# ahmetaa/fast-dnn

Hardware: AMD Instinct MI355X
Metric: acoustic frames/sec (whole node), 7x2048->8000 nnet (higher is better)
Workload: dtype int8 (u8 activations x s8 weights -> int32; fp32 layer 0 and soft-max)

## Files before the change

### fast-dnn_amd/csrc/fdnn_l0s.hip

```cpp
#include <atomic>
#include <cmath>
#include <cstdlib>
#include <limits>
#include <type_traits>
#include <vector>

#include "fdnn_device.hpp"
#include "fdnn_kernels.hpp"

namespace fdnn {

namespace {

#ifndef FDNN_L0S_DEBUG
#define FDNN_L0S_DEBUG 0
#endif
constexpr float kU = 5.9604645e-8f;
constexpr int kSplitW = 32;

[[maybe_unused]] __device__ __forceinline__ bool split_tile_of_block(int node_tiles, int frame_tiles, int &bx, int &by) {
  const int b = blockIdx.x, xcd = b & 7, slot = b >> 3;
  bx = slot % node_tiles;
  by = xcd + 8 * (slot / node_tiles);
  return by < frame_tiles;
}

constexpr int kDigFrames = 8;
__global__ __launch_bounds__(256) void l0_digits_kernel(L0Params p, int KC, int J, int JP) {
  extern __shared__ __attribute__((aligned(16))) float dig_smem[];
  const int D = p.D, ld = D + 1;
  float *xs = dig_smem;
  float *cf_s = dig_smem + kDigFrames * ld;
  const int tid = threadIdx.x, f0 = blockIdx.x * kDigFrames;
  if (blockIdx.x == 0 && tid < 2) p.glist_count[tid] = 0u;
  const int quads = D >> 2;
  {
    float4 raw[4], sh[4], sc[4];
    int rowq[4];
#pragma unroll
    for (int it = 0; it < 4; ++it) {
      const int i = tid + it * 256;
      const int row = i / quads, q = i - row * quads, f = f0 + row;
      const bool in = i < kDigFrames * quads;
      rowq[it] = in ? row * ld + 4 * q : -1;
      raw[it] = make_float4(0.f, 0.f, 0.f, 0.f);
      sh[it] = raw[it];
      sc[it] = raw[it];
      if (in && f < p.n) {
        raw[it] = *reinterpret_cast<const float4 *>(p.x + static_cast<size_t>(f) * D + 4 * q);
        sh[it] = *reinterpret_cast<const float4 *>(p.shift + 4 * q);
        sc[it] = *reinterpret_cast<const float4 *>(p.scale + 4 * q);
      }
    }
#pragma unroll
    for (int it = 0; it < 4; ++it) {
      if (rowq[it] < 0) continue;
      float *dst = xs + rowq[it];
      dst[0] = (raw[it].x + sh[it].x) * sc[it].x;
      dst[1] = (raw[it].y + sh[it].y) * sc[it].y;
      dst[2] = (raw[it].z + sh[it].z) * sc[it].z;
      dst[3] = (raw[it].w + sh[it].w) * sc[it].w;
    }
  }
  __syncthreads();
  {
    const int row = tid >> 5, sub = tid & 31;
    float mx = 0.0f, s2 = 0.0f, s1 = 0.0f;
    int bad = 0;
    float vals[16];
#pragma unroll
    for (int it = 0; it < 16; ++it) vals[it] = sub + 32 * it < D ? xs[row * ld + sub + 32 * it] : 0.0f;
#pragma unroll
    for (int it = 0; it < 16; ++it) {
      const float v = vals[it], a = fabsf(v);
      bad |= !(a < 3.0e38f);
      mx = fmaxf(mx, a);
      s2 = fmaf(v, v, s2);
      s1 += a;
    }
#pragma unroll
    for (int off = 1; off < 32; off <<= 1) {
      mx = fmaxf(mx, __shfl_xor(mx, off));
      s2 += __shfl_xor(s2, off);
      s1 += __shfl_xor(s1, off);
      bad |= __shfl_xor(bad, off);
    }
    if (sub == 0) {
      const bool degenerate = bad || mx > 1.0e18f || (mx != 0.0f && mx < 1.0e-18f);
      const float cf = (mx == 0.0f || degenerate) ? 1.0f : 8355000.0f / mx;
      cf_s[row] = degenerate ? 0.0f : cf;
      const float fD = static_cast<float>(D);
      const float slack = 1.001f + 2.0f * kU * fD;
      const float n1X = (cf * s1 * slack + fD) * 1.001f;
      const float n1X1 = n1X * (1.0f / 65536.0f) + 0.502f * fD;
      const float m = static_cast<float>(JP / 32 + 1);
      const float a_f = kU * (kSplitW + 3) * m * 0.502f * n1X1 + 2.3283064e-10f * (0.5f * n1X + 0.5f * fD) + kU * 256.0f * fD;
      const int f = f0 + row;
      if (f < p.n_ld) {
        p.xstat[f] = 65536.0f / cf;
        p.xstat[p.n_ld + f] = sqrtf(s2) * (1.00001f + 2.0f * kU * fD);
        p.xstat[2 * p.n_ld + f] = degenerate ? __builtin_inff() : 256.0f * a_f * 1.002f;
      }
    }
  }
  __syncthreads();
  for (int idx = tid; idx < kDigFrames * KC * 2; idx += 256) {
    const int row = idx & 7, hh = (idx >> 3) & 1, kc = idx >> 4;
    const float cf = cf_s[row];
    uint32_t d1[4], d2[4], d3[4];
#pragma unroll
    for (int e4 = 0; e4 < 4; ++e4) {
      uint32_t w1 = 0, w2 = 0, w3 = 0;
#pragma unroll
      for (int e = 0; e < 4; ++e) {
        const int pp = kc * 32 + hh * 16 + e4 * 4 + e;
        const int c = (pp >= JP) + (pp >= 2 * JP) + (pp >= 3 * JP), j = pp - c * JP;
        const float v = j < J ? xs[row * ld + 4 * j + c] : 0.0f;
        const int X = static_cast<int>(rintf(v * cf));
        const int x3 = (X << 24) >> 24, r = (X - x3) >> 8, x2 = (r << 24) >> 24, x1 = (r - x2) >> 8;
        w1 |= static_cast<uint32_t>(x1 & 0xff) << (8 * e);
        w2 |= static_cast<uint32_t>(x2 & 0xff) << (8 * e);
        w3 |= static_cast<uint32_t>(x3 & 0xff) << (8 * e);
      }
      d1[e4] = w1; d2[e4] = w2; d3[e4] = w3;
    }
    const int f = f0 + row;
    if (f >= p.n_ld) continue;
    const size_t blocks = static_cast<size_t>(p.n_ld >> 5);
#pragma unroll
    for (int pl = 0; pl < 3; ++pl) {
      const uint32_t *d = pl == 0 ? d1 : pl == 1 ? d2 : d3;
      char *base = reinterpret_cast<char *>(p.xd) + ((static_cast<size_t>(kc) * 3 + pl) * blocks + (f >> 5)) * 1024 + hh * 512 + (f & 31) * 16;
      *reinterpret_cast<uint4 *>(base) = make_uint4(d[0], d[1], d[2], d[3]);
    }
  }
}

constexpr int kSTF = 128, kSStages = 3;
template <int WN>
struct SplitCfg {
  static constexpr int TN = 64 * WN, NW = 4 * WN, THREADS = 64 * NW;
  static constexpr int PIECES = 12 + 6 * WN;
  static constexpr int STAGE = PIECES * 1024;
  static constexpr int RING = STAGE * kSStages;
  static constexpr int HALF_OFF = RING;
  static constexpr int STAT_OFF = RING + 11 * 1024;
  static constexpr int LDS = STAT_OFF + 3 * 1024;
  static constexpr int TS = TN + 16;
  static constexpr int PPW = (PIECES + NW - 1) / NW;
  static_assert(kSTF * TS + 16 + 2 * kL0ScreenCap <= RING, "epilogue tile and flag list must fit in the dead ring");
};
static_assert(4 * kLut2Size <= 11 * 1024, "half-step table area");

template <int WN, bool DBG = false>
__global__ __launch_bounds__(256 * WN, 3 - WN) void l0_split_kernel(L0Params p, int KC, int CPC) {
#if defined(__HIP_DEVICE_COMPILE__)
  using Cfg = SplitCfg<WN>;
  constexpr int kSTN = Cfg::TN, kSStage = Cfg::STAGE, kSTS = Cfg::TS, kSHalfOff = Cfg::HALF_OFF, kSStatOff = Cfg::STAT_OFF, NW = Cfg::NW;
  extern __shared__ __attribute__((aligned(16))) char smem[];
  const int tid = threadIdx.x, lane = tid & 63;
  const int wave = __builtin_amdgcn_readfirstlane(tid >> 6);
  const int l32 = lane & 31, h = lane >> 5;
  const int wf = wave & 3, wn = wave >> 2;
  const int node_tiles = p.h_ld / kSTN, frame_tiles = (p.n_rows + kSTF - 1) / kSTF;
  int bx, by;
  if (!split_tile_of_block(node_tiles, frame_tiles, bx, by)) return;
  const int f0 = by * kSTF, n0 = bx * kSTN;
  const int xblocks = p.n_ld >> 5, wblocks = p.h_ld >> 5;
#ifdef FDNN_L0S_CLK
  long long tc[12];
  tc[0] = __builtin_readcyclecounter();
#define L0S_TS(i) tc[i] = __builtin_readcyclecounter()
#else
#define L0S_TS(i)
#endif

  {
    const __amdgpu_buffer_rsrc_t rsrc_half =
        __builtin_amdgcn_make_buffer_rsrc(const_cast<uint32_t *>(p.luthalf), 0, (4 * kLut2Size + 15) & ~15, 0x00020000);
#pragma unroll
    for (int i = 0; i < 14; ++i) {
      if (i % NW != wave) continue;
      if (i < 11) {
        __builtin_amdgcn_raw_ptr_buffer_load_lds(rsrc_half, FDNN_LDS_PTR(smem + kSHalfOff + i * 1024), 16, lane * 16, i * 1024, 0, 0);
      } else {
        const int q = i - 11;
        const __amdgpu_buffer_rsrc_t rsrc_st =
            __builtin_amdgcn_make_buffer_rsrc(const_cast<float *>(p.xstat + static_cast<size_t>(q) * p.n_ld + f0), 0, kSTF * 4, 0x00020000);
        __builtin_amdgcn_raw_ptr_buffer_load_lds(rsrc_st, FDNN_LDS_PTR(smem + kSStatOff + q * 1024), 16, lane * 16, 0, 0, 0);
      }
    }
  }
  const __amdgpu_buffer_rsrc_t rsrc_x =
      __builtin_amdgcn_make_buffer_rsrc(const_cast<int8_t *>(p.xd), 0, static_cast<unsigned>(KC) * 3u * static_cast<unsigned>(xblocks) * 1024u, 0x00020000);
  const __amdgpu_buffer_rsrc_t rsrc_w = __builtin_amdgcn_make_buffer_rsrc(
      const_cast<int8_t *>(p.wd), 0, static_cast<unsigned>(KC) * 3u * static_cast<unsigned>(wblocks) * 1024u, 0x00020000);
  const int voff = lane * 16;
  const int my_pieces = (Cfg::PIECES - wave + NW - 1) / NW;
  auto stage_piece = [&](int kc, int buf, int t) {
    char *base = smem + buf * kSStage;
    const int i = wave + NW * t;
    if (i >= Cfg::PIECES) return;
    if (i < 12) {
      const int pl = i >> 2, q = i & 3;
      __builtin_amdgcn_raw_ptr_buffer_load_lds(rsrc_x, FDNN_LDS_PTR(base + i * 1024), 16, voff, ((kc * 3 + pl) * xblocks + (f0 >> 5) + q) * 1024, 0, 0);
    } else {
      const int j = i - 12, pl = j / (2 * WN), q = j % (2 * WN);
      __builtin_amdgcn_raw_ptr_buffer_load_lds(rsrc_w, FDNN_LDS_PTR(base + i * 1024), 16, voff, ((kc * 3 + pl) * wblocks + (n0 >> 5) + q) * 1024, 0, 0);
    }
  };
  auto stage = [&](int kc, int buf) {
#pragma unroll
    for (int t = 0; t < Cfg::PPW; ++t) stage_piece(kc, buf, t);
  };
  auto wait_stages = [&](int stages) {
    if (stages == 0) {
      asm volatile("s_waitcnt vmcnt(0) lgkmcnt(0)" ::: "memory");
    } else if (Cfg::PIECES % NW == 0) {
      if (stages == 1)
        asm volatile("s_waitcnt vmcnt(%0) lgkmcnt(0)" ::"n"(Cfg::PPW) : "memory");
      else
        asm volatile("s_waitcnt vmcnt(%0) lgkmcnt(0)" ::"n"(2 * Cfg::PPW) : "memory");
    } else if (my_pieces == Cfg::PPW) {
      if (stages == 1)
        asm volatile("s_waitcnt vmcnt(%0) lgkmcnt(0)" ::"n"(Cfg::PPW) : "memory");
      else
        asm volatile("s_waitcnt vmcnt(%0) lgkmcnt(0)" ::"n"(2 * Cfg::PPW) : "memory");
    } else {
      if (stages == 1)
        asm volatile("s_waitcnt vmcnt(%0) lgkmcnt(0)" ::"n"(Cfg::PPW - 1) : "memory");
      else
        asm volatile("s_waitcnt vmcnt(%0) lgkmcnt(0)" ::"n"(2 * (Cfg::PPW - 1)) : "memory");
    }
  };
  stage(0, 0);
  stage(1, 1);
  stage(2, 2);
  asm volatile("" ::: "memory");

  constexpr int kP0Off = 0x40000000;
  v16i P0[2], P1[2], P2[2];
  uint32_t A[2][16];
#pragma unroll
  for (int s = 0; s < 2; ++s)
#pragma unroll
    for (int r = 0; r < 16; ++r) {
      P0[s][r] = kP0Off; P1[s][r] = 0; P2[s][r] = 0;
      A[s][r] = 0u;
    }
  auto chain_end = [&](int s) {
#pragma unroll
    for (int r = 0; r < 16; ++r) {
      P1[s][r] += P0[s][r] << 8;
      P0[s][r] = kP0Off;
    }
  };
  v4i xa[2][3], wb[2][3][2];
  auto load_plane = [&](int buf, int set, int pl) {
    const char *sb = smem + buf * kSStage;
    xa[set][pl] = *reinterpret_cast<const v4i *>(sb + (pl * 4 + wf) * 1024 + lane * 16);
#pragma unroll
    for (int s = 0; s < 2; ++s) wb[set][pl][s] = *reinterpret_cast<const v4i *>(sb + 12288 + (pl * 2 * WN + wn * 2 + s) * 1024 + lane * 16);
  };
  auto load_frags = [&](int buf, int set) {
#pragma unroll
    for (int pl = 0; pl < 3; ++pl) load_plane(buf, set, pl);
  };
  auto sample_part = [&](int ss, int r0, int r1, bool on) {
    if ((FDNN_L0S_DEBUG & 1) || !on) return;
#pragma unroll
    for (int r = r0; r < r1; ++r) asm volatile("v_sad_u32 %0, %1, 2.0, %0" : "+v"(A[ss][r]) : "v"(P0[ss][r]));
  };
#define FDNN_L0S_FENCE __builtin_amdgcn_sched_barrier(0)
  auto mfma_group = [&](int set, int s, int ss, bool on, auto x0, auto x1, auto x2, auto x3, auto x4) {
    FDNN_L0S_FENCE;
    P0[s] = __builtin_amdgcn_mfma_i32_32x32x32_i8(xa[set][0], wb[set][0][s], P0[s], 0, 0, 0);
    if (FDNN_L0S_DEBUG & 2) {
      sample_part(ss, 0, 16, on);
      x0(); x1(); x2(); x3(); x4();
      return;
    }
    FDNN_L0S_FENCE;
    sample_part(ss, 0, 3, on);
    x0();
    FDNN_L0S_FENCE;
    P1[s] = __builtin_amdgcn_mfma_i32_32x32x32_i8(xa[set][0], wb[set][1][s], P1[s], 0, 0, 0);
    FDNN_L0S_FENCE;
    sample_part(ss, 3, 6, on);
    x1();
    FDNN_L0S_FENCE;
    P2[s] = __builtin_amdgcn_mfma_i32_32x32x32_i8(xa[set][0], wb[set][2][s], P2[s], 0, 0, 0);
    FDNN_L0S_FENCE;
    sample_part(ss, 6, 9, on);
    x2();
    FDNN_L0S_FENCE;
    P1[s] = __builtin_amdgcn_mfma_i32_32x32x32_i8(xa[set][1], wb[set][0][s], P1[s], 0, 0, 0);
    FDNN_L0S_FENCE;
    sample_part(ss, 9, 12, on);
    x3();
    FDNN_L0S_FENCE;
    P2[s] = __builtin_amdgcn_mfma_i32_32x32x32_i8(xa[set][1], wb[set][1][s], P2[s], 0, 0, 0);
    FDNN_L0S_FENCE;
    sample_part(ss, 12, 16, on);
    x4();
    FDNN_L0S_FENCE;
    P2[s] = __builtin_amdgcn_mfma_i32_32x32x32_i8(xa[set][2], wb[set][0][s], P2[s], 0, 0, 0);
    FDNN_L0S_FENCE;
  };
  auto nothing = [] {};

  wait_stages(2);
  __builtin_amdgcn_s_barrier();
  asm volatile("" ::: "memory");
  load_frags(0, 0);
  L0S_TS(1);
  auto chunk = [&](int kc, auto set_c, auto first_c, bool chain_start) {
    constexpr int set = decltype(set_c)::value;
    constexpr bool first = decltype(first_c)::value;
    if (chain_start) chain_end(0);
    mfma_group(set, 0, 1, !first, nothing, nothing, nothing, nothing, nothing);
    const bool more = kc + 1 < KC, refill = kc + 3 < KC && !(FDNN_L0S_DEBUG & 8);
    if (more) {
      wait_stages(kc + 2 < KC ? 1 : 0);
      if (!(FDNN_L0S_DEBUG & 16)) __builtin_amdgcn_s_barrier();
      asm volatile("" ::: "memory");
    }
    if (chain_start) chain_end(1);
    const int nb = (kc + 1) % 3;
    mfma_group(
        set, 1, 0, true, [&] { if (more && !(FDNN_L0S_DEBUG & 32)) load_plane(nb, set ^ 1, 0); if (refill) stage_piece(kc + 3, kc % 3, 0); },
        [&] { if (more && !(FDNN_L0S_DEBUG & 32)) load_plane(nb, set ^ 1, 1); if (refill) stage_piece(kc + 3, kc % 3, 1); },
        [&] { if (more && !(FDNN_L0S_DEBUG & 32)) load_plane(nb, set ^ 1, 2); if (refill) stage_piece(kc + 3, kc % 3, 2); },
        [&] { if (refill && Cfg::PPW > 3) stage_piece(kc + 3, kc % 3, 3); }, [&] { if (refill && Cfg::PPW > 4) stage_piece(kc + 3, kc % 3, 4); });
  };
  using C0 = std::integral_constant<int, 0>;
  using C1 = std::integral_constant<int, 1>;
  chunk(0, C0{}, std::true_type{}, false);
  chunk(1, C1{}, std::false_type{}, false);
  for (int kc = 2, in_chain = 2; kc < KC; kc += 2, in_chain += 2) {
    const bool chain_start = in_chain == CPC;
    if (chain_start) in_chain = 0;
    chunk(kc, C0{}, std::false_type{}, chain_start);
    chunk(kc + 1, C1{}, std::false_type{}, false);
  }
  sample_part(1, 0, 16, true);
  chain_end(0);
  chain_end(1);
  L0S_TS(2);

  __syncthreads();
  const char *half_b = smem + kSHalfOff + 4 * kLut2Half;
  const float *rf_s = reinterpret_cast<const float *>(smem + kSStatOff);
  const float *xn_s = rf_s + 256, *af_s = rf_s + 512;
  uint8_t *tile = reinterpret_cast<uint8_t *>(smem);
  uint32_t *scr_n = reinterpret_cast<uint32_t *>(tile + kSTF * kSTS);
  uint16_t *scr_l = reinterpret_cast<uint16_t *>(tile + kSTF * kSTS + 16);
  if (tid == 0) *scr_n = 0;
  const float fD = static_cast<float>(p.D);
  const float c2 = 1.001f * (0.5f * fD * fD + 2.0f * fD) * kU;
  const float kA = 1.00001f * 256.0f * 1.002f * kU * (kSplitW + 3);
  const float kS = 100.001f * 1.002f * kU * (kSplitW / 2 + 2 + c2);
  float bias100[2], rn100[2], kSw2[2], bn2[2], eb2[2];
  bool node_in[2];
#pragma unroll
  for (int s = 0; s < 2; ++s) {
    const int node = n0 + wn * 64 + s * 32 + l32;
    node_in[s] = node < p.H;
    const float b = node_in[s] ? p.bias[node] : 0.0f;
    bias100[s] = 100.0f * b;
    rn100[s] = 100.0f * (node_in[s] ? p.wstat[node] : 0.0f);
    kSw2[s] = kS * (node_in[s] ? p.wstat[p.h_ld + node] : 0.0f);
    bn2[s] = 1.00001f * (node_in[s] ? p.wstat[2 * p.h_ld + node] : 0.0f);
    eb2[s] = 100.001f * 10.0f * kU * fabsf(b);
  }
  uint32_t valid = 0;
#pragma unroll
  for (int r = 0; r < 16; ++r) {
    const bool row_in = f0 + wf * 32 + 8 * (r >> 2) + 4 * h + (r & 3) < p.n;
    valid |= (row_in && node_in[0] ? 1u : 0u) << r;
    valid |= (row_in && node_in[1] ? 1u : 0u) << (16 + r);
  }
  float tt[2][16], sg[2][16];
  uint32_t ent[2][16];
#pragma unroll
  for (int r = 0; r < 16; ++r) {
    const float rf = rf_s[wf * 32 + 8 * (r >> 2) + 4 * h + (r & 3)];
#pragma unroll
    for (int s = 0; s < 2; ++s) {
      const float v = fmaf(static_cast<float>(P2[s][r]), 0.00390625f, static_cast<float>(P1[s][r]));
      sg[s][r] = rf * rn100[s];
      tt[s][r] = fmaf(v, sg[s][r], bias100[s]);
      const int u = lut2_clamp(static_cast<int>(tt[s][r] + tt[s][r]));
      ent[s][r] = *reinterpret_cast<const uint32_t *>(half_b + 4 * u);
    }
  }
  uint32_t scr_mask = 0;
#pragma unroll
  for (int r = 0; r < 16; ++r) {
    const int row = wf * 32 + 8 * (r >> 2) + 4 * h + (r & 3);
    const float xn = xn_s[row], af = af_s[row];
#pragma unroll
    for (int s = 0; s < 2; ++s) {
      const float t = tt[s][r], sig = sg[s][r];
      tile[row * kSTS + wn * 64 + s * 32 + l32] = static_cast<uint8_t>(ent[s][r]);
      if (!(FDNN_L0S_DEBUG & 4)) {
        const float e = __builtin_amdgcn_fractf(t) - 0.5f;
        const float Dd = fmaf(fabsf(t), 12.0f * kU, fmaf(sig, fmaf(kA, static_cast<float>(A[s][r]), af + bn2[s]), fmaf(kSw2[s], xn, eb2[s]))) + 1e-30f;
        const float gate = __builtin_bit_cast(float, ent[s][r] & 0xffff0000u);
        const float m = fmaxf(fmaxf(fabsf(e), gate), fabsf(t) - 641.0f);
        const bool flag = !(m > Dd) | !(fabsf(t) < 1.0e9f);
        scr_mask |= flag ? (1u << (16 * s + r)) : 0u;
        if (DBG && ((valid >> (16 * s + r)) & 1u)) {
          const size_t o = static_cast<size_t>(f0 + row) * p.H + (n0 + wn * 64 + s * 32 + l32);
          p.dbg_t[o] = t;
          p.dbg_dd[o] = Dd;
        }
      }
    }
  }
  scr_mask &= valid;
  L0S_TS(3);
  __syncthreads();
  L0S_TS(4);
  {
    const int mine = __popc(scr_mask);
    int incl = mine;
#pragma unroll
    for (int off = 1; off < 64; off <<= 1) {
      const int v = __shfl_up(incl, off);
      if (lane >= off) incl += v;
    }
    const int wave_total = __shfl(incl, 63);
    if (wave_total) {
      uint32_t base = 0;
      if (lane == 63) base = atomicAdd(scr_n, static_cast<uint32_t>(wave_total));
      base = __shfl(base, 63);
      uint32_t at = base + static_cast<uint32_t>(incl - mine);
      uint32_t m = scr_mask;
      while (m) {
        const int i = __ffs(m) - 1;
        m &= m - 1;
        const int r = i & 15, sb2 = i >> 4;
        const int row = wf * 32 + 8 * (r >> 2) + 4 * h + (r & 3), col = wn * 64 + sb2 * 32 + l32;
        if (at < static_cast<uint32_t>(kL0ScreenCap)) scr_l[at] = static_cast<uint16_t>(row * kSTN + col);
        ++at;
      }
    }
  }
#pragma unroll
  for (int q = 0; q < kSTF * (kSTN / 16) / Cfg::THREADS; ++q) {
    const int item = tid + q * Cfg::THREADS, row = item / (kSTN / 16), c16 = (item % (kSTN / 16)) * 16;
    const int f = f0 + row;
    if (f < p.n_rows && n0 + c16 < p.H)
      *reinterpret_cast<uint4 *>(p.act_out + static_cast<size_t>(f) * p.act_ld + n0 + c16) = *reinterpret_cast<const uint4 *>(tile + row * kSTS + c16);
  }
  __syncthreads();
  {
    const uint32_t cnt = *scr_n;
    uint32_t *gbase_s = scr_n + 1;
    if (tid == 0) {
      uint32_t gb = 0xffffffffu, fill_from = 0xffffffffu;
      if (cnt != 0 && cnt <= static_cast<uint32_t>(kL0ScreenCap)) {
        gb = atomicAdd(p.glist_count, cnt);
        if (gb + cnt > static_cast<uint32_t>(p.glist_cap)) {
          fill_from = gb;
          gb = 0xffffffffu;
        }
      }
      if (cnt != 0 && gb == 0xffffffffu) {
        p.scr_count[by * (p.h_ld / 128) + (n0 >> 7)] = cnt;
        atomicAdd(p.glist_count + 1, 1u);
      }
      *gbase_s = gb;
      gbase_s[1] = fill_from;
    }
    __syncthreads();
    const uint32_t gb = *gbase_s, fill_from = gbase_s[1];
    if (fill_from < static_cast<uint32_t>(p.glist_cap))
      for (uint32_t i = fill_from + tid; i < static_cast<uint32_t>(p.glist_cap); i += Cfg::THREADS) p.glist[i] = make_uint2(0xffffffffu, 0xffffffffu);
    if (gb != 0xffffffffu)
      for (uint32_t i = tid; i < cnt; i += Cfg::THREADS) {
        const uint32_t e = scr_l[i];
        p.glist[gb + i] = make_uint2(static_cast<uint32_t>(f0) + e / kSTN, static_cast<uint32_t>(n0) + e % kSTN);
      }
  }
#ifdef FDNN_L0S_CLK
  L0S_TS(5);
  if (p.scr_stats && lane == 0 && wave == 0 && (blockIdx.x == 0 || blockIdx.x == gridDim.x / 2 + 3)) {
    unsigned long long *o = p.scr_stats + 4 + (blockIdx.x == 0 ? 0 : 12);
    for (int i = 0; i < 6; ++i) o[i] = static_cast<unsigned long long>(tc[i] - tc[0]);
  }
#endif
#endif
}

}

size_t l0_split_half_bytes() { return (4 * size_t(kLut2Size) + 15) & ~size_t(15); }

void l0_split_build_weights(const float *w, const float *wnorm, const uint8_t *lut2, int H, int D, int h_ld, std::vector<int8_t> *planes,
                            std::vector<float> *stat, std::vector<uint32_t> *half) {
  const int J = D / 4, JP = l0_split_chain_pad(D);
  planes->assign(l0_split_plane_bytes(D, h_ld), 0);
  stat->assign(static_cast<size_t>(3) * h_ld, 0.0f);
  half->assign(l0_split_half_bytes() / 4, 0);
  auto at = [&](int u) { return lut2[lut2_clamp(u) + kLut2Half]; };
  for (int u = -kLut2Half; u <= kLut2Half; ++u) {
    const int mag = u < 0 ? -u : u;
    bool same;
    if (u == 0)
      same = at(0) == at(1) && at(0) == at(-1);
    else
      same = at(u) == at(u < 0 ? -(mag ^ 1) : (mag ^ 1));
    (*half)[u + kLut2Half] = at(u) | (same ? 0x3e800000u : 0u);
  }
  const size_t blocks = static_cast<size_t>(h_ld / 32);
  const double u = std::ldexp(1.0, -24);
  const double m = static_cast<double>(JP / 32 + 1);
  for (int n = 0; n < H; ++n) {
    const float *row = w + static_cast<size_t>(n) * D;
    double mx = 0.0;
    bool bad = false;
    for (int k = 0; k < D; ++k) {
      const double a = std::fabs(static_cast<double>(row[k]));
      if (!(a < 3.0e38)) bad = true;
      if (a > mx) mx = a;
    }
    const bool degenerate = bad || mx > 1.0e18 || (mx != 0.0 && mx < 1.0e-18);
    const float cn = (mx == 0.0 || degenerate) ? 1.0f : static_cast<float>(8355000.0 / mx);
    double n1W = 0.0, n1W2 = 0.0, n1W3 = 0.0;
    for (int pp = 0; pp < 4 * JP; ++pp) {
      const int c = pp / JP, j = pp - c * JP, k = 4 * j + c;
      if (j >= J) continue;
      const long W = degenerate ? 0 : std::lrint(static_cast<double>(row[k]) * static_cast<double>(cn));
      n1W += static_cast<double>(W < 0 ? -W : W);
      const int x3 = static_cast<int8_t>(W & 0xff), r = static_cast<int>((W - x3) >> 8), x2 = static_cast<int8_t>(r & 0xff), x1 = (r - x2) >> 8;
      n1W2 += std::abs(x2);
      n1W3 += std::abs(x3);
      const int digit[3] = {x1, x2, x3};
      const int kc = pp >> 5, hh = (pp >> 4) & 1, e = pp & 15;
      for (int pl = 0; pl < 3; ++pl)
        (*planes)[((static_cast<size_t>(kc) * 3 + pl) * blocks + (n >> 5)) * 1024 + hh * 512 + (n & 31) * 16 + e] = static_cast<int8_t>(digit[pl]);
    }
    const double b_n = (u * (kSplitW + 3) * m * 0.502 * n1W / 65536.0 + std::ldexp(0.5 * n1W, -32) + std::ldexp(128.0 * (n1W2 + n1W3), -24) +
                        std::ldexp(128.0 * n1W3, -32)) * 1.002;
    auto up = [](double v) {
      float f = static_cast<float>(v);
      if (static_cast<double>(f) < v) f = std::nextafter(f, std::numeric_limits<float>::infinity());
      return f;
    };
    (*stat)[n] = 256.0f / cn;
    (*stat)[static_cast<size_t>(h_ld) + n] = wnorm[n];
    (*stat)[static_cast<size_t>(2) * h_ld + n] = degenerate ? std::numeric_limits<float>::infinity() : up(256.0 * b_n);
  }
}

static_assert(kSTF == 128, "fdnn_select.hpp: choose_l0 counts this kernel's 128-frame tiles");
static_assert(kSTF == kL0TileFrames, "fdnn_ctx_layout.hpp counts the planes' rows and the per-tile counters in these tiles");
void launch_l0_split(const L0Params &p, int wn_cfg, hipStream_t s) {
  const int KC = l0_split_chunks(p.D), J = p.D / 4, JP = l0_split_chain_pad(p.D);
  static std::atomic<unsigned long long> attr_set{0};
  int dev = 0;
  (void)hipGetDevice(&dev);
  const unsigned long long dev_bit = 1ull << (dev & 63);
  const int dig_lds = (kDigFrames * (p.D + 1) + kDigFrames) * 4;
  if (!(attr_set.load(std::memory_order_acquire) & dev_bit)) {
    (void)hipFuncSetAttribute(reinterpret_cast<const void *>(l0_split_kernel<1>), hipFuncAttributeMaxDynamicSharedMemorySize, SplitCfg<1>::LDS);
    (void)hipFuncSetAttribute(reinterpret_cast<const void *>(l0_split_kernel<2>), hipFuncAttributeMaxDynamicSharedMemorySize, SplitCfg<2>::LDS);
    attr_set.fetch_or(dev_bit, std::memory_order_release);
  }
  const int frame_tiles = (p.n_rows + kSTF - 1) / kSTF;
  const int dig_rows = frame_tiles * kSTF;
  note_launch(kLn_l0_digits);
  hipLaunchKernelGGL(l0_digits_kernel, dim3(dig_rows / kDigFrames), dim3(256), dig_lds, s, p, KC, J, JP);
  if (p.dbg_t != nullptr && p.dbg_dd != nullptr) {
    (void)hipFuncSetAttribute(reinterpret_cast<const void *>(l0_split_kernel<2, true>), hipFuncAttributeMaxDynamicSharedMemorySize, SplitCfg<2>::LDS);
    note_launch(kLn_l0_split_n128_probe);
    hipLaunchKernelGGL((l0_split_kernel<2, true>), dim3(static_cast<unsigned>(p.h_ld / 128) * ((frame_tiles + 7) / 8) * 8), dim3(512), SplitCfg<2>::LDS, s, p, KC, JP / 32);
    return;
  }
  note_launch(wn_cfg == 2 ? kLn_l0_split_n128 : kLn_l0_split_n64);
  if (wn_cfg == 2)
    hipLaunchKernelGGL(l0_split_kernel<2>, dim3(static_cast<unsigned>(p.h_ld / 128) * ((frame_tiles + 7) / 8) * 8), dim3(512), SplitCfg<2>::LDS, s, p, KC, JP / 32);
  else
    hipLaunchKernelGGL(l0_split_kernel<1>, dim3(static_cast<unsigned>(p.h_ld / 64) * ((frame_tiles + 7) / 8) * 8), dim3(256), SplitCfg<1>::LDS, s, p, KC, JP / 32);
}

}
```

Baseline: 15.72 million.

## Rewrite layer-0 digit kernel with chain-major LDS layout and byte-perm packing

Templates the layer-0 digit-splitting kernel on chain padding and wave count, and stores normalized inputs in LDS already split into the four chains, so the split stage reads contiguous float4 vectors instead of strided scalars. Global loads switch to bounds-checked buffer loads. The per-element shift/mask digit extraction becomes an offset add plus v_perm byte shuffles. Block size drops from 256 to 256 threads in four waves with a templated barrier, and the NaN/Inf check is folded into the sum test. The change limits supported D to chains of at most 128 positions.

```diff
diff --git a/fast-dnn_amd/csrc/fdnn_l0s.hip b/fast-dnn_amd/csrc/fdnn_l0s.hip
--- a/fast-dnn_amd/csrc/fdnn_l0s.hip
+++ b/fast-dnn_amd/csrc/fdnn_l0s.hip
@@ -26,67 +26,102 @@
 }
 
 constexpr int kDigFrames = 8;
-__global__ __launch_bounds__(256) void l0_digits_kernel(L0Params p, int KC, int J, int JP) {
+constexpr int kDigChainPad = 8;
+constexpr int kDigWaves = 4;
+template <int JP>
+struct DigCfg {
+  static constexpr int CS = JP + kDigChainPad, RS = 4 * CS, KC = JP / 8;
+  static constexpr int LDS = (kDigFrames * RS + kDigFrames) * 4;
+};
+template <int W>
+__device__ __forceinline__ void dig_sync() {
+  if (W == 1) {
+    __builtin_amdgcn_fence(__ATOMIC_RELEASE, "wavefront");
+    __builtin_amdgcn_wave_barrier();
+    __builtin_amdgcn_fence(__ATOMIC_ACQUIRE, "wavefront");
+  } else {
+    __syncthreads();
+  }
+}
+template <int JP, int W>
+__global__ __launch_bounds__(64 * W) void l0_digits_kernel(L0Params p) {
+  using Cfg = DigCfg<JP>;
+  constexpr int cs = Cfg::CS, rs = Cfg::RS, KC = Cfg::KC;
+  constexpr int RW = kDigFrames / W, PW = kDigFrames / 2 / W;
+  constexpr int H2 = JP > 64 ? 2 : 1;
+  static_assert((JP == 64 || JP == 128) && (W == 1 || W == 2 || W == 4), "D <= 496: chains of at most 128 positions");
   extern __shared__ __attribute__((aligned(16))) float dig_smem[];
-  const int D = p.D, ld = D + 1;
   float *xs = dig_smem;
-  float *cf_s = dig_smem + kDigFrames * ld;
-  const int tid = threadIdx.x, f0 = blockIdx.x * kDigFrames;
-  if (blockIdx.x == 0 && tid < 2) p.glist_count[tid] = 0u;
-  const int quads = D >> 2;
+  float *cf_s = dig_smem + kDigFrames * rs;
+  const int D = p.D, J = D >> 2;
+  const int lane = threadIdx.x & 63, w = W == 1 ? 0 : __builtin_amdgcn_readfirstlane(threadIdx.x >> 6);
+  const int f0 = blockIdx.x * kDigFrames;
+  if (blockIdx.x == 0 && threadIdx.x < 2) p.glist_count[threadIdx.x] = 0u;
   {
-    float4 raw[4], sh[4], sc[4];
-    int rowq[4];
-#pragma unroll
-    for (int it = 0; it < 4; ++it) {
-      const int i = tid + it * 256;
-      const int row = i / quads, q = i - row * quads, f = f0 + row;
-      const bool in = i < kDigFrames * quads;
-      rowq[it] = in ? row * ld + 4 * q : -1;
-      raw[it] = make_float4(0.f, 0.f, 0.f, 0.f);
-      sh[it] = raw[it];
-      sc[it] = raw[it];
-      if (in && f < p.n) {
-        raw[it] = *reinterpret_cast<const float4 *>(p.x + static_cast<size_t>(f) * D + 4 * q);
-        sh[it] = *reinterpret_cast<const float4 *>(p.shift + 4 * q);
-        sc[it] = *reinterpret_cast<const float4 *>(p.scale + 4 * q);
-      }
-    }
-#pragma unroll
-    for (int it = 0; it < 4; ++it) {
-      if (rowq[it] < 0) continue;
-      float *dst = xs + rowq[it];
-      dst[0] = (raw[it].x + sh[it].x) * sc[it].x;
-      dst[1] = (raw[it].y + sh[it].y) * sc[it].y;
-      dst[2] = (raw[it].z + sh[it].z) * sc[it].z;
-      dst[3] = (raw[it].w + sh[it].w) * sc[it].w;
-    }
-  }
-  __syncthreads();
+    const int rows_in = min(kDigFrames, p.n - f0);
+    const __amdgpu_buffer_rsrc_t rsrc_x = __builtin_amdgcn_make_buffer_rsrc(const_cast<float *>(p.x) + static_cast<size_t>(rows_in > 0 ? f0 : 0) * D, 0,
+                                                                            rows_in > 0 ? rows_in * D * 4 : 0, 0x00020000);
+    const __amdgpu_buffer_rsrc_t rsrc_sh = __builtin_amdgcn_make_buffer_rsrc(const_cast<float *>(p.shift), 0, D * 4, 0x00020000);
+    const __amdgpu_buffer_rsrc_t rsrc_sc = __builtin_amdgcn_make_buffer_rsrc(const_cast<float *>(p.scale), 0, D * 4, 0x00020000);
+    float4 raw[RW][H2], sh[H2], sc[H2];
+#pragma unroll
+    for (int h2 = 0; h2 < H2; ++h2) {
+      const int q = lane + 64 * h2;
+      const int voff = q < J ? 16 * q : 0x40000000;
+#pragma unroll
+      for (int i = 0; i < RW; ++i)
+        raw[i][h2] = __builtin_bit_cast(float4, __builtin_amdgcn_raw_buffer_load_b128(rsrc_x, voff + (w + W * i) * D * 4, 0, 0));
+      sh[h2] = __builtin_bit_cast(float4, __builtin_amdgcn_raw_buffer_load_b128(rsrc_sh, 16 * q, 0, 0));
+      sc[h2] = __builtin_bit_cast(float4, __builtin_amdgcn_raw_buffer_load_b128(rsrc_sc, 16 * q, 0, 0));
+    }
+    float *dst0 = xs + w * rs + lane;
+#pragma unroll
+    for (int i = 0; i < RW; ++i) {
+      const bool in = f0 + w + W * i < p.n;
+#pragma unroll
+      for (int h2 = 0; h2 < H2; ++h2) {
+        float *dst = dst0 + W * i * rs + 64 * h2;
+        dst[0] = in ? (raw[i][h2].x + sh[h2].x) * sc[h2].x : 0.0f;
+        dst[cs] = in ? (raw[i][h2].y + sh[h2].y) * sc[h2].y : 0.0f;
+        dst[2 * cs] = in ? (raw[i][h2].z + sh[h2].z) * sc[h2].z : 0.0f;
+        dst[3 * cs] = in ? (raw[i][h2].w + sh[h2].w) * sc[h2].w : 0.0f;
+      }
+    }
+  }
+  dig_sync<W>();
   {
-    const int row = tid >> 5, sub = tid & 31;
-    float mx = 0.0f, s2 = 0.0f, s1 = 0.0f;
-    int bad = 0;
-    float vals[16];
-#pragma unroll
-    for (int it = 0; it < 16; ++it) vals[it] = sub + 32 * it < D ? xs[row * ld + sub + 32 * it] : 0.0f;
-#pragma unroll
-    for (int it = 0; it < 16; ++it) {
-      const float v = vals[it], a = fabsf(v);
-      bad |= !(a < 3.0e38f);
-      mx = fmaxf(mx, a);
-      s2 = fmaf(v, v, s2);
-      s1 += a;
-    }
-#pragma unroll
-    for (int off = 1; off < 32; off <<= 1) {
-      mx = fmaxf(mx, __shfl_xor(mx, off));
-      s2 += __shfl_xor(s2, off);
-      s1 += __shfl_xor(s1, off);
-      bad |= __shfl_xor(bad, off);
-    }
-    if (sub == 0) {
-      const bool degenerate = bad || mx > 1.0e18f || (mx != 0.0f && mx < 1.0e-18f);
+    const int sub = lane & 31, half = lane >> 5;
+    float tmx[PW], ts2[PW], ts1[PW];
+    const float *src0 = xs + (2 * w + half) * rs + (sub & 3) * cs + (sub >> 2);
+#pragma unroll
+    for (int i = 0; i < PW; ++i) {
+      const float *src = src0 + 2 * W * i * rs;
+      float mx = 0.0f, s2 = 0.0f, s1 = 0.0f;
+      float vals[JP / 8];
+#pragma unroll
+      for (int it = 0; it < JP / 8; ++it) vals[it] = sub + 32 * it < D ? src[8 * it] : 0.0f;
+#pragma unroll
+      for (int it = 0; it < JP / 8; ++it) {
+        const float v = vals[it], a = fabsf(v);
+        mx = fmaxf(mx, a);
+        s2 = fmaf(v, v, s2);
+        s1 += a;
+      }
+#pragma unroll
+      for (int off = 1; off < 32; off <<= 1) {
+        mx = fmaxf(mx, __shfl_xor(mx, off));
+        s2 += __shfl_xor(s2, off);
+        s1 += __shfl_xor(s1, off);
+      }
+      tmx[i] = mx, ts2[i] = s2, ts1[i] = s1;
+    }
+    float mx = tmx[0], s2 = ts2[0], s1 = ts1[0];
+#pragma unroll
+    for (int i = 1; i < PW; ++i)
+      if (sub == i) mx = tmx[i], s2 = ts2[i], s1 = ts1[i];
+    if (sub < PW) {
+      const int row = 2 * (w + W * sub) + half;
+      const bool degenerate = !(s1 == s1) || mx > 1.0e18f || (mx != 0.0f && mx < 1.0e-18f);
       const float cf = (mx == 0.0f || degenerate) ? 1.0f : 8355000.0f / mx;
       cf_s[row] = degenerate ? 0.0f : cf;
       const float fD = static_cast<float>(D);
@@ -103,30 +138,31 @@
       }
     }
   }
-  __syncthreads();
-  for (int idx = tid; idx < kDigFrames * KC * 2; idx += 256) {
-    const int row = idx & 7, hh = (idx >> 3) & 1, kc = idx >> 4;
-    const float cf = cf_s[row];
+  dig_sync<W>();
+  const int row = lane & 7, hh = (lane >> 3) & 1, f = f0 + row;
+  const float cf = cf_s[row];
+  const size_t blocks = static_cast<size_t>(p.n_ld >> 5);
+#pragma unroll
+  for (int kc0 = 0; kc0 < KC; kc0 += 4 * W) {
+    const int kc = kc0 + 4 * w + (lane >> 4);
+    if (W > 1 && 4 * W > KC && kc >= KC) break;
+    const int pp = kc * 32 + hh * 16, c = pp / JP, j = pp - c * JP;
+    const float4 *src = reinterpret_cast<const float4 *>(xs + row * rs + c * cs + j);
+    const float4 v4[4] = {src[0], src[1], src[2], src[3]};
     uint32_t d1[4], d2[4], d3[4];
 #pragma unroll
     for (int e4 = 0; e4 < 4; ++e4) {
-      uint32_t w1 = 0, w2 = 0, w3 = 0;
-#pragma unroll
-      for (int e = 0; e < 4; ++e) {
-        const int pp = kc * 32 + hh * 16 + e4 * 4 + e;
-        const int c = (pp >= JP) + (pp >= 2 * JP) + (pp >= 3 * JP), j = pp - c * JP;
-        const float v = j < J ? xs[row * ld + 4 * j + c] : 0.0f;
-        const int X = static_cast<int>(rintf(v * cf));
-        const int x3 = (X << 24) >> 24, r = (X - x3) >> 8, x2 = (r << 24) >> 24, x1 = (r - x2) >> 8;
-        w1 |= static_cast<uint32_t>(x1 & 0xff) << (8 * e);
-        w2 |= static_cast<uint32_t>(x2 & 0xff) << (8 * e);
-        w3 |= static_cast<uint32_t>(x3 & 0xff) << (8 * e);
-      }
-      d1[e4] = w1; d2[e4] = w2; d3[e4] = w3;
-    }
-    const int f = f0 + row;
+      const float v[4] = {v4[e4].x, v4[e4].y, v4[e4].z, v4[e4].w};
+      uint32_t Y[4];
+#pragma unroll
+      for (int e = 0; e < 4; ++e) Y[e] = static_cast<uint32_t>(static_cast<int>(rintf(v[e] * cf)) + 0x8080);
+      const uint32_t lo01 = __builtin_amdgcn_perm(Y[1], Y[0], 0x05010400u), lo23 = __builtin_amdgcn_perm(Y[3], Y[2], 0x05010400u);
+      const uint32_t hi01 = __builtin_amdgcn_perm(Y[1], Y[0], 0x0c0c0602u), hi23 = __builtin_amdgcn_perm(Y[3], Y[2], 0x0c0c0602u);
+      d1[e4] = __builtin_amdgcn_perm(hi23, hi01, 0x05040100u);
+      d2[e4] = __builtin_amdgcn_perm(lo23, lo01, 0x07060302u) ^ 0x80808080u;
+      d3[e4] = __builtin_amdgcn_perm(lo23, lo01, 0x05040100u) ^ 0x80808080u;
+    }
     if (f >= p.n_ld) continue;
-    const size_t blocks = static_cast<size_t>(p.n_ld >> 5);
 #pragma unroll
     for (int pl = 0; pl < 3; ++pl) {
       const uint32_t *d = pl == 0 ? d1 : pl == 1 ? d2 : d3;
@@ -558,12 +594,11 @@
 static_assert(kSTF == 128, "fdnn_select.hpp: choose_l0 counts this kernel's 128-frame tiles");
 static_assert(kSTF == kL0TileFrames, "fdnn_ctx_layout.hpp counts the planes' rows and the per-tile counters in these tiles");
 void launch_l0_split(const L0Params &p, int wn_cfg, hipStream_t s) {
-  const int KC = l0_split_chunks(p.D), J = p.D / 4, JP = l0_split_chain_pad(p.D);
+  const int KC = l0_split_chunks(p.D), JP = l0_split_chain_pad(p.D);
   static std::atomic<unsigned long long> attr_set{0};
   int dev = 0;
   (void)hipGetDevice(&dev);
   const unsigned long long dev_bit = 1ull << (dev & 63);
-  const int dig_lds = (kDigFrames * (p.D + 1) + kDigFrames) * 4;
   if (!(attr_set.load(std::memory_order_acquire) & dev_bit)) {
     (void)hipFuncSetAttribute(reinterpret_cast<const void *>(l0_split_kernel<1>), hipFuncAttributeMaxDynamicSharedMemorySize, SplitCfg<1>::LDS);
     (void)hipFuncSetAttribute(reinterpret_cast<const void *>(l0_split_kernel<2>), hipFuncAttributeMaxDynamicSharedMemorySize, SplitCfg<2>::LDS);
@@ -572,7 +607,10 @@
   const int frame_tiles = (p.n_rows + kSTF - 1) / kSTF;
   const int dig_rows = frame_tiles * kSTF;
   note_launch(kLn_l0_digits);
-  hipLaunchKernelGGL(l0_digits_kernel, dim3(dig_rows / kDigFrames), dim3(256), dig_lds, s, p, KC, J, JP);
+  if (JP == 64)
+    hipLaunchKernelGGL((l0_digits_kernel<64, kDigWaves>), dim3(dig_rows / kDigFrames), dim3(64 * kDigWaves), DigCfg<64>::LDS, s, p);
+  else
+    hipLaunchKernelGGL((l0_digits_kernel<128, kDigWaves>), dim3(dig_rows / kDigFrames), dim3(64 * kDigWaves), DigCfg<128>::LDS, s, p);
   if (p.dbg_t != nullptr && p.dbg_dd != nullptr) {
     (void)hipFuncSetAttribute(reinterpret_cast<const void *>(l0_split_kernel<2, true>), hipFuncAttributeMaxDynamicSharedMemorySize, SplitCfg<2>::LDS);
     note_launch(kLn_l0_split_n128_probe);
```

Result: no change. 15.79 million (median of 2 runs) (+0.5%).
